# ducha-aiki/affnet

Hardware: AMD Instinct MI355X
Metric: keypoints/sec (detect+AffNet+OriNet+HardNet) per image, 2000 kp @1024x768 (higher is better)
Workload: dtype f32

## Files before the change

affnet_amd/csrc/cnn32.hip:

```cpp
#include <math.h>
#include <stdlib.h>

#include <algorithm>
#include <type_traits>

#include "common.h"

#include "cnn_mfma.h"
#include "shape_filter.h"

#define HEAD_PART_AFF 32
#define HEAD_PART_ORI 144
template <int TM>
__device__ __forceinline__ void head_partials(const float* __restrict__ hw, const f32x4 (&bias)[1], const f32x4 (&acc)[TM][1],
                                              float* __restrict__ part, int wave, int lane) {
    constexpr int MT = 4, MG = MT / TM;
    const int mg = wave % MG, ng = wave / MG;
    const int n = lane & 15, g = lane >> 4;
    const int c4 = ng * 16 + 4 * g;
    f32x4 v[TM];
#pragma unroll
    for (int i = 0; i < TM; ++i) {
        v[i] = acc[i][0] + bias[0];
        v[i].x = fmaxf(v[i].x, 0.0f); v[i].y = fmaxf(v[i].y, 0.0f); v[i].z = fmaxf(v[i].z, 0.0f); v[i].w = fmaxf(v[i].w, 0.0f);
// ... 159 lines not shown
    static constexpr int NB1 = 2, NB3 = 1;
    static constexpr int offset(int layer) { return layer == 1 ? 0 : (layer == 3 ? U1 : U1 + U3); }
    static constexpr int floats(int layer) { return layer == 1 ? U1 : (layer == 3 ? U3 : U5); }
};

__global__ __launch_bounds__(256) void wino_derive_u_kernel(const float* __restrict__ packed, int w1, int w3, int w5, float* __restrict__ U) {
    int e = blockIdx.x * 256 + threadIdx.x;
    if (e >= Wino16::PAIRS) return;
    const int l = e >= 256 + 1024 ? 5 : (e >= 256 ? 3 : 1);
    const int ch = 8 << ((l + 1) >> 1);
    const float* src = packed + (l == 5 ? w5 : (l == 3 ? w3 : w1));
    float* dst = U + Wino16::offset(l);
    e -= l == 5 ? 256 + 1024 : (l == 3 ? 256 : 0);
    const int n = (e >> 2) % ch, c = (e >> 2) / ch * 4 + (e & 3);
    float g[9], u[16];
#pragma unroll
    for (int t = 0; t < 9; ++t) g[t] = src[w_tap_index(t, c, n, ch, ch)];
    wino_weight_transform(g, u);
#pragma unroll
    for (int xi = 0; xi < 16; ++xi) dst[w_tap_index(xi, c, n, ch, ch)] = u[xi];
}

template <int CB>
struct TrunkLds {
    static constexpr int ACT = (CB / 4) * LayC0::PSG;
    static constexpr int PATCH = WP32 * WP32;
    static constexpr int RED = 256;
    static constexpr int TOTAL = ACT + PATCH + RED;
};

template <int KIND, int NW>
struct TrunkShape {
    static constexpr int CB = (KIND == AFFNET_NET_HARDNET) ? 32 : 16;
    static constexpr int NTHR = NW * 64;
    static constexpr int T1M = (CB == 16) ? 8 : 64 / NW, T1N = CB / 16;
    static constexpr int T2M = (CB == 16) ? 4 : 64 / NW, T2N = 1;
    static constexpr int T4M = (CB == 16) ? 2 : 32 / NW, T4N = 1;
    static constexpr int AREG = (NW == 8 && CB == 32) ? 128 : 48;
    static constexpr int G2 = pick_groups(CB, T2M, T2N, 32, AREG), G3 = pick_groups(2 * CB, T2M, T2N, 32, AREG);
    static constexpr int G4 = pick_groups(2 * CB, T4M, T4N, 32, AREG), G5 = pick_groups(4 * CB, T4M, T4N, 32, AREG);
};

template <int C, typename L, int NTHR>
__device__ __forceinline__ void dump_planes(const float* act, float* dst) {
    constexpr int H = L::H;
    for (int i = threadIdx.x; i < C * H * H; i += NTHR) {
        const int c = i / (H * H), r = i - c * H * H, y = r / H, x = r - y * H;
        dst[i] = act[L::at(c, y, x)];
    }
}

template <int CB>
struct SplitLays {
    typedef LayQ<16, 32, 34, CB, 0, 3> LQH;
    typedef LayQ<16, 32, 34, CB, 16, 3> LQH2;
    using LR0 = LayR<32, 32, 34, CB, 0>;
    using LR0H = LayR<16, 32, 34, CB, 0, 34>;
    using LR1 = LayR<32, 32, 34, CB, 16>;
    using LR1H = LayR<16, 32, 34, CB, 16, 34>;
    static_assert(LR0::BYTES <= TrunkLds<CB>::ACT * 4 && LR1::BYTES <= TrunkLds<CB>::ACT * 4 && LR0H::GS == LR0::GS && LR1H::GS == LR1::GS, "whole-patch split layouts");
    static_assert(LQH::BYTES <= TrunkLds<CB>::ACT * 4 && LQH2::BYTES <= TrunkLds<CB>::ACT * 4, "pre-split layouts must fit the activation buffer");
};

template <int KIND, int NW, bool STAMPS, int S3 = 0>
__global__ __launch_bounds__(NW * 64, (KIND == AFFNET_NET_HARDNET) ? NW / 4 : 4) void cnn32_trunk_kernel(CnnArgs a, PyrSrc ps) {
    static_assert(S3 == 0 || S3 == 2 || S3 == 3, "S3 = number of terms of the split arithmetic");
    using S = TrunkShape<KIND, NW>;
    constexpr int CB = S::CB, NTHR = S::NTHR;
    static_assert((CB / 4) * LayC1::PSG <= TrunkLds<CB>::ACT && (CB / 2) * LayC3::PSG <= TrunkLds<CB>::ACT, "LDS layout");
    __shared__ __attribute__((aligned(16))) float lds[TrunkLds<CB>::TOTAL];
    float* act = lds;
    float* patch = lds + TrunkLds<CB>::ACT;
    float* red = patch + TrunkLds<CB>::PATCH;
    const int n = a.count ? min(a.count[blockIdx.y], a.n_max) : a.n_max;
    const int prow = blockIdx.x + a.row_begin;
    if (KIND == AFFNET_NET_AFFNET && a.shape_cnt && blockIdx.x == 0 && threadIdx.x == 0) {
        int32_t* c = a.shape_cnt + (size_t)blockIdx.y * CNT_TOTAL;
        if (a.shape_op == 1) { c[CNT_SURVIVED] = 0; c[CNT_SURVIVED1] = 0; c[CNT_AFF_EVAL] = 0; }
        else if (a.shape_op == 2) c[CNT_SURVIVED1] = c[CNT_SURVIVED];
    }
    if (prow >= n || lazy_skip(a.skip_cnt, a.skip_n, blockIdx.y, CNT_SURVIVED)) return;
    const size_t pidx = (size_t)blockIdx.y * a.n_max + prow;
    const int tid = threadIdx.x, wave = tid >> 6, lane = tid & 63;
    if (KIND == AFFNET_NET_HARDNET) __builtin_amdgcn_s_setprio(3);
    CNN_STAMP(0);
    if (STAMPS && a.dbg_time && lane == 0) {
        a.dbg_time[((size_t)pidx * NW + wave) * 32 + 14] = __builtin_amdgcn_s_getreg((31 << 11) | 4);
        a.dbg_time[((size_t)pidx * NW + wave) * 32 + 15] = __builtin_amdgcn_s_getreg((31 << 11) | 20);
    }
    float w0[3][S::T1N];
    f32x4 bias0[S::T1N];
    conv0_load_w<NW, CB, S::T1M, S::T1N>(a.packed + a.off.w[0], a.packed + a.off.b[0], w0, bias0, wave, lane);
    f32x4 b1[1][S::T1N];
    f32x4 Ur[4];
    if constexpr (S3 == 0 && KIND == AFFNET_NET_AFFNET) prefetch_b0<NW, CB, 32, S::T1M, S::T1N, 1>(a.packed + a.off.w[1], b1, wave, lane);
    if constexpr (S3 == 0 && KIND == AFFNET_NET_ORINET) wino_prefetch_u_row<NW, CB, CB, 32, Wino16::NB1>(a.wino_u, Ur, wave, lane);

    constexpr int PPT = 1024 / NTHR;
    constexpr int RPT = 32 / PPT;
    float v[PPT];
    if (a.patches) {
        const float* src = a.patches + pidx * 1024;
#pragma unroll
        for (int q = 0; q < PPT; ++q) v[q] = src[tid + q * NTHR];
    } else {
        int o = a.ids[3 * pidx], l = a.ids[3 * pidx + 1];
        o = o < 0 ? 0 : (o >= ps.t.n_octaves ? ps.t.n_octaves - 1 : o);
        l = l < 0 ? 0 : (l >= ps.t.n_levels ? ps.t.n_levels - 1 : l);
        const float* img = ps.t.lvl[o][l] + blockIdx.y * ps.t.img_stride;
        const int h = ps.t.h[o], w = ps.t.w[o];
        const float* L = a.lafs + 6 * pidx;
        const float m = (float)(h < w ? h : w);
        const float t00 = L[0] * m, t01 = L[1] * m, t02 = L[2] * (float)w;
        const float t10 = L[3] * m, t11 = L[4] * m, t12 = L[5] * (float)h;
#pragma unroll
        for (int q = 0; q < PPT; ++q)
            v[q] = aff_sample_bilinear(img, h, w, t00, t01, t02, t10, t11, t12, ps.base[tid & 31], ps.base[(tid >> 5) + q * RPT]);
    }
    CNN_STAMP(16);
    if (tid < 4 * 33) {
        const int e = tid;
        const int y = e < 34 ? 0 : (e < 68 ? 33 : 1 + ((e - 68) >> 1)), x = e < 34 ? e : (e < 68 ? e - 34 : ((e - 68) & 1) * 33);
        patch[y * WP32 + x] = 0.0f;
    }
    if constexpr (S3 == 0) zero_halo<LayC0, NTHR>(act, CB);
    else if constexpr (S3 == 2) zero_halo_q<typename SplitLays<CB>::LR0, NTHR>(act);
    else zero_halo_q<typename SplitLays<CB>::LQH, NTHR>(act);
    float sum = 0.f;
#pragma unroll
    for (int q = 0; q < PPT; ++q) sum += v[q];
    const float mean = block_sum<NW>(sum, red) * (1.0f / 1024.0f);
    CNN_STAMP(17);
    float sq = 0.f;
#pragma unroll
    for (int q = 0; q < PPT; ++q) { v[q] -= mean; sq += v[q] * v[q]; }
    const float var = block_sum<NW>(sq, red + NW) * (1.0f / 1023.0f);
    const float sd = sqrtf(var) + 1e-7f;
    CNN_STAMP(18);
#pragma unroll
    for (int q = 0; q < PPT; ++q) patch[((tid >> 5) + q * RPT + 1) * WP32 + (tid & 31) + 1] = v[q] / sd;
    __syncthreads();
    CNN_STAMP(1);

    if constexpr (S3 == 0 && KIND == AFFNET_NET_HARDNET) {
        constexpr int T1M = S::T1M, T1N = S::T1N, T2M = S::T2M, T2N = S::T2N, T4M = S::T4M, T4N = S::T4N;
        constexpr int NB1 = (16 * 16 / 16) * (CB / 16) / NW, NB3 = (8 * 8 / 16) * (2 * CB / 16) / NW, NB5 = (4 * 4 / 16) * (4 * CB / 16) / NW;

        f32x4 Up[2][4];
        f32x4 Uw[16];
        {
            f32x4 acc[T1M][T1N];
            conv0_mfma<NW, CB, T1M, T1N>(patch, w0, bias0, acc, wave, lane);
            CNN_STAMP(19);
            store_tiles_lds<CB, LayC0, T1M, T1N, false>(act, bias0, acc, wave, lane);
            CNN_STAMP(20);
            wino_prefetch_u_pair<NW, CB, CB, 32, NB1>(a.packed + a.off.w_wino[0], Up, wave, lane);
            __syncthreads();
        }
        if (STAMPS && a.dbg_layer == 0) { dump_planes<CB, LayC0, NTHR>(act, a.dbg_out); return; }
        CNN_STAMP(2);

        f32x4 b2[S::G2][T2N];
        f32x4 bias2[T2N];
        {
            f32x4 y[NB1][4], bw[NB1];
            __builtin_amdgcn_s_setprio(0);
            conv3x3_wino_mfma_pair_rows<NW, CB, CB, LayC0, NB1>(act, a.packed + a.off.w_wino[0], Up, y, wave, lane);
            __builtin_amdgcn_s_setprio(3);
            CNN_STAMP(3);
            prefetch_b0<NW, 2 * CB, 16, T2M, T2N, S::G2>(a.packed + a.off.w[2], b2, wave, lane);
            prefetch_bias<NW, 16, T2M, T2N>(a.packed + a.off.b[2], bias2, wave, lane);
            wino_bias<NW, 32, CB, NB1>(a.packed + a.off.b[1], bw, wave, lane);
            __syncthreads();
            CNN_STAMP(21);
            zero_halo<LayC1, NTHR>(act, CB);
            wino_store_lds<CB, LayC1, NB1>(act, bw, y, wave, lane);
            CNN_STAMP(22);
            __syncthreads();
            CNN_STAMP(4);
        }
        if (STAMPS && a.dbg_layer == 1) { dump_planes<CB, LayC1, NTHR>(act, a.dbg_out); return; }

        {
            f32x4 acc[T2M][T2N];
            __builtin_amdgcn_s_setprio(0);
            conv3x3_mfma<NW, CB, 2 * CB, LayC1, 2, T2M, T2N, S::G2>(act, a.packed + a.off.w[2], b2, acc, wave, lane);
            __builtin_amdgcn_s_setprio(3);
            CNN_STAMP(5);
            wino_prefetch_u_pair<NW, 2 * CB, 2 * CB, 16, NB3>(a.packed + a.off.w_wino[1], Up, wave, lane);
            __syncthreads();
            zero_halo<LayC2, NTHR>(act, 2 * CB);
            store_tiles_lds<2 * CB, LayC2, T2M, T2N>(act, bias2, acc, wave, lane);
            __syncthreads();
            CNN_STAMP(6);
        }
        if (STAMPS && a.dbg_layer == 2) { dump_planes<2 * CB, LayC2, NTHR>(act, a.dbg_out); return; }

        f32x4 b4[S::G4][T4N];
        f32x4 bias4[T4N];
        {
            f32x4 y[NB3][4], bw[NB3];
            __builtin_amdgcn_s_setprio(0);
            conv3x3_wino_mfma_pair_rows<NW, 2 * CB, 2 * CB, LayC2, NB3>(act, a.packed + a.off.w_wino[1], Up, y, wave, lane);
            __builtin_amdgcn_s_setprio(3);
            CNN_STAMP(7);
            prefetch_b0<NW, 4 * CB, 8, T4M, T4N, S::G4>(a.packed + a.off.w[4], b4, wave, lane);
            prefetch_bias<NW, 8, T4M, T4N>(a.packed + a.off.b[4], bias4, wave, lane);
            wino_bias<NW, 16, 2 * CB, NB3>(a.packed + a.off.b[3], bw, wave, lane);
            __syncthreads();
            zero_halo<LayC3, NTHR>(act, 2 * CB);
            wino_store_lds<2 * CB, LayC3, NB3>(act, bw, y, wave, lane);
            __syncthreads();
            CNN_STAMP(8);
        }
        if (STAMPS && a.dbg_layer == 3) { dump_planes<2 * CB, LayC3, NTHR>(act, a.dbg_out); return; }

        {
            f32x4 acc[T4M][T4N];
            __builtin_amdgcn_s_setprio(0);
            conv3x3_mfma<NW, 2 * CB, 4 * CB, LayC3, 2, T4M, T4N, S::G4>(act, a.packed + a.off.w[4], b4, acc, wave, lane);
            __builtin_amdgcn_s_setprio(3);
            CNN_STAMP(9);
            wino_prefetch_u<NW, 4 * CB, 4 * CB, 8, NB5>(a.packed + a.off.w_wino[2], Uw, wave, lane);
            __syncthreads();
            zero_halo<LayC4, NTHR>(act, 4 * CB);
            store_tiles_lds<4 * CB, LayC4, T4M, T4N>(act, bias4, acc, wave, lane);
            __syncthreads();
            CNN_STAMP(10);
        }
        if (STAMPS && a.dbg_layer == 4) { dump_planes<4 * CB, LayC4, NTHR>(act, a.dbg_out); return; }

        f32x4 y[NB5][4], bw[NB5];
        __builtin_amdgcn_s_setprio(0);
        static_assert(NB5 == 1 && (4 * CB / 16) * 4096 <= TrunkLds<CB>::ACT, "conv5: one pass per wave, V of the layer fits the activation buffer");
        conv3x3_wino_mfma_shared_v<NW, 4 * CB, 4 * CB, LayC4>(act, a.packed + a.off.w_wino[2], Uw, y, wave, lane);
        __builtin_amdgcn_s_setprio(3);
        CNN_STAMP(11);
        wino_bias<NW, 8, 4 * CB, NB5>(a.packed + a.off.b[5], bw, wave, lane);
        if (!STAMPS || a.dbg_layer < 0) {
            wino_store_global<4 * CB, 8, NB5>(a.out + pidx * (64 * 4 * CB), bw, y, wave, lane);
            CNN_STAMP(13);
            return;
        }
        __syncthreads();
        wino_store_lds<4 * CB, LayC5, NB5>(act, bw, y, wave, lane);
        __syncthreads();
        CNN_STAMP(12);
        if (STAMPS && a.dbg_layer == 5) { dump_planes<4 * CB, LayC5, NTHR>(act, a.dbg_out); return; }
    } else if constexpr (S3 == 0) {
        constexpr int T1M = S::T1M, T1N = S::T1N, T2M = S::T2M, T2N = S::T2N, T4M = S::T4M, T4N = S::T4N;
        static_assert(NW == 8 && CB == 16, "Wino16 describes the 16-channel trunks on 8 waves");
        f32x4 b4[S::G4][T4N];
        f32x4 bias4[T4N];
        if constexpr (KIND == AFFNET_NET_ORINET) {
            constexpr int NB1 = Wino16::NB1, NB3 = Wino16::NB3;
            {
                f32x4 acc[T1M][T1N];
                conv0_mfma<NW, CB, T1M, T1N>(patch, w0, bias0, acc, wave, lane);
                CNN_STAMP(19);
                store_tiles_lds<CB, LayC0, T1M, T1N, false>(act, bias0, acc, wave, lane);
                CNN_STAMP(20);
                __syncthreads();
            }
            if (STAMPS && a.dbg_layer == 0) { dump_planes<CB, LayC0, NTHR>(act, a.dbg_out); return; }
            CNN_STAMP(2);

            f32x4 b2[S::G2][T2N];
            f32x4 bias2[T2N];
            {
                f32x4 y[NB1][4], bw[NB1];
                conv3x3_wino_mfma_rows<NW, CB, CB, LayC0, NB1>(act, a.wino_u, Ur, y, wave, lane);
                CNN_STAMP(3);
                prefetch_b0<NW, 2 * CB, 16, T2M, T2N, S::G2>(a.packed + a.off.w[2], b2, wave, lane);
                prefetch_bias<NW, 16, T2M, T2N>(a.packed + a.off.b[2], bias2, wave, lane);
                wino_bias<NW, 32, CB, NB1>(a.packed + a.off.b[1], bw, wave, lane);
                __syncthreads();
                CNN_STAMP(21);
                zero_halo<LayC1, NTHR>(act, CB);
                wino_store_lds<CB, LayC1, NB1>(act, bw, y, wave, lane);
                CNN_STAMP(22);
                __syncthreads();
                CNN_STAMP(4);
            }
            if (STAMPS && a.dbg_layer == 1) { dump_planes<CB, LayC1, NTHR>(act, a.dbg_out); return; }

            {
                f32x4 acc[T2M][T2N];
                conv3x3_mfma<NW, CB, 2 * CB, LayC1, 2, T2M, T2N, S::G2>(act, a.packed + a.off.w[2], b2, acc, wave, lane);
                CNN_STAMP(5);
                wino_prefetch_u_row<NW, 2 * CB, 2 * CB, 16, NB3>(a.wino_u + Wino16::offset(3), Ur, wave, lane);
                __syncthreads();
                zero_halo<LayC2, NTHR>(act, 2 * CB);
                store_tiles_lds<2 * CB, LayC2, T2M, T2N>(act, bias2, acc, wave, lane);
                __syncthreads();
                CNN_STAMP(6);
            }
            if (STAMPS && a.dbg_layer == 2) { dump_planes<2 * CB, LayC2, NTHR>(act, a.dbg_out); return; }

            {
                f32x4 y[NB3][4], bw[NB3];
                conv3x3_wino_mfma_rows<NW, 2 * CB, 2 * CB, LayC2, NB3>(act, a.wino_u + Wino16::offset(3), Ur, y, wave, lane);
                CNN_STAMP(7);
                prefetch_b0<NW, 4 * CB, 8, T4M, T4N, S::G4>(a.packed + a.off.w[4], b4, wave, lane);
                prefetch_bias<NW, 8, T4M, T4N>(a.packed + a.off.b[4], bias4, wave, lane);
                wino_bias<NW, 16, 2 * CB, NB3>(a.packed + a.off.b[3], bw, wave, lane);
                __syncthreads();
                zero_halo<LayC3, NTHR>(act, 2 * CB);
                wino_store_lds<2 * CB, LayC3, NB3>(act, bw, y, wave, lane);
                __syncthreads();
                CNN_STAMP(8);
            }
            if (STAMPS && a.dbg_layer == 3) { dump_planes<2 * CB, LayC3, NTHR>(act, a.dbg_out); return; }

        } else {
            static_assert(T1M * 8 > S::AREG, "conv1: two A sets of T1M float4 do not fit -> rolling single set (conv3x3_mfma_roll)");
            f32x4 bias1[T1N];
            {
                f32x4 acc[T1M][T1N];
                conv0_mfma<NW, CB, T1M, T1N>(patch, w0, bias0, acc, wave, lane);
                CNN_STAMP(19);
                prefetch_bias<NW, 32, T1M, T1N>(a.packed + a.off.b[1], bias1, wave, lane);
                store_tiles_lds<CB, LayC0, T1M, T1N, false>(act, bias0, acc, wave, lane);
                CNN_STAMP(20);
                __syncthreads();
            }
            if (STAMPS && a.dbg_layer == 0) { dump_planes<CB, LayC0, NTHR>(act, a.dbg_out); return; }
            CNN_STAMP(2);

            f32x4 b2[S::G2][T2N];
            f32x4 bias2[T2N];
            {
                f32x4 acc[T1M][T1N];
                conv3x3_mfma_roll<NW, CB, CB, LayC0, 1, T1M, T1N>(act, a.packed + a.off.w[1], b1, acc, wave, lane);
                CNN_STAMP(3);
                prefetch_b0<NW, 2 * CB, 16, T2M, T2N, S::G2>(a.packed + a.off.w[2], b2, wave, lane);
                prefetch_bias<NW, 16, T2M, T2N>(a.packed + a.off.b[2], bias2, wave, lane);
                __syncthreads();
                CNN_STAMP(21);
                zero_halo<LayC1, NTHR>(act, CB);
                store_tiles_lds<CB, LayC1, T1M, T1N>(act, bias1, acc, wave, lane);
                CNN_STAMP(22);
                __syncthreads();
                CNN_STAMP(4);
            }
            if (STAMPS && a.dbg_layer == 1) { dump_planes<CB, LayC1, NTHR>(act, a.dbg_out); return; }

            f32x4 b3[S::G3][T2N];
            f32x4 bias3[T2N];
            {
                f32x4 acc[T2M][T2N];
                conv3x3_mfma<NW, CB, 2 * CB, LayC1, 2, T2M, T2N, S::G2>(act, a.packed + a.off.w[2], b2, acc, wave, lane);
                CNN_STAMP(5);
                prefetch_b0<NW, 2 * CB, 16, T2M, T2N, S::G3>(a.packed + a.off.w[3], b3, wave, lane);
                prefetch_bias<NW, 16, T2M, T2N>(a.packed + a.off.b[3], bias3, wave, lane);
                __syncthreads();
                zero_halo<LayC2, NTHR>(act, 2 * CB);
                store_tiles_lds<2 * CB, LayC2, T2M, T2N>(act, bias2, acc, wave, lane);
                __syncthreads();
                CNN_STAMP(6);
            }
            if (STAMPS && a.dbg_layer == 2) { dump_planes<2 * CB, LayC2, NTHR>(act, a.dbg_out); return; }

            {
                f32x4 acc[T2M][T2N];
                conv3x3_mfma<NW, 2 * CB, 2 * CB, LayC2, 1, T2M, T2N, S::G3>(act, a.packed + a.off.w[3], b3, acc, wave, lane);
                CNN_STAMP(7);
                prefetch_b0<NW, 4 * CB, 8, T4M, T4N, S::G4>(a.packed + a.off.w[4], b4, wave, lane);
                prefetch_bias<NW, 8, T4M, T4N>(a.packed + a.off.b[4], bias4, wave, lane);
                __syncthreads();
                zero_halo<LayC3, NTHR>(act, 2 * CB);
                store_tiles_lds<2 * CB, LayC3, T2M, T2N>(act, bias3, acc, wave, lane);
                __syncthreads();
                CNN_STAMP(8);
            }
            if (STAMPS && a.dbg_layer == 3) { dump_planes<2 * CB, LayC3, NTHR>(act, a.dbg_out); return; }

        }

        f32x4 b5[S::G5][T4N];
        f32x4 bias5[T4N];
        {
            f32x4 acc[T4M][T4N];
            conv3x3_mfma<NW, 2 * CB, 4 * CB, LayC3, 2, T4M, T4N, S::G4>(act, a.packed + a.off.w[4], b4, acc, wave, lane);
            CNN_STAMP(9);
            if constexpr (KIND == AFFNET_NET_ORINET) {
                wino5_prefetch_u(a.wino_u + Wino16::offset(5), Ur, wave, lane);
            } else {
                prefetch_b0<NW, 4 * CB, 8, T4M, T4N, S::G5>(a.packed + a.off.w[5], b5, wave, lane);
                prefetch_bias<NW, 8, T4M, T4N>(a.packed + a.off.b[5], bias5, wave, lane);
            }
            __syncthreads();
// ... 900 lines not shown
```

affnet_amd/csrc/cnn_mfma.h:

```cpp
#pragma once
#include <math.h>
#include <stdlib.h>

#include "common.h"
#include "weights_layout.h"

typedef float f32x4 __attribute__((ext_vector_type(4)));

typedef __attribute__((address_space(3))) const f32x4 LdsF4;
__device__ __forceinline__ unsigned lds_byte_addr(const float* p) {
    return (unsigned)(size_t)(__attribute__((address_space(3))) const float*)p;
}
__device__ __forceinline__ f32x4 lds_read4(unsigned byte_addr) { return *(LdsF4*)(size_t)byte_addr; }

typedef unsigned u32x4 __attribute__((ext_vector_type(4)));
__device__ __forceinline__ __amdgpu_buffer_rsrc_t weight_rsrc(const float* base, int n_floats) {
    return __builtin_amdgcn_make_buffer_rsrc(const_cast<float*>(base), 0, n_floats * 4, 0x00020000);
}
__device__ __forceinline__ f32x4 buf_read4(__amdgpu_buffer_rsrc_t r, int lane_byte_off, int uniform_byte_off) {
    return __builtin_bit_cast(f32x4, __builtin_amdgcn_raw_buffer_load_b128(r, lane_byte_off, uniform_byte_off, 0));
}

template <int H_, int WP_, int PSG_>
struct Lay {
// ... 757 lines not shown
        const int p = (mg * TM + i) * 16 + m;
        const int base = (p >> 5) * WP32 + (p & 31);
        float av[3];
#pragma unroll
        for (int s3 = 0; s3 < 3; ++s3) av[s3] = patch[base + toff[s3]];
#pragma unroll
        for (int s3 = 0; s3 < 3; ++s3)
#pragma unroll
            for (int j = 0; j < TN; ++j) acc[i][j] = __builtin_amdgcn_mfma_f32_16x16x4f32(b[s3][j], av[s3], acc[i][j], 0, 0, 0);
    }
}

template <int COUT, typename LO, int TM, int TN, bool ADD_BIAS = true>
__device__ __forceinline__ void store_tiles_lds(float* act, const f32x4 (&bias)[TN], const f32x4 (&acc)[TM][TN], int wave, int lane) {
    constexpr int HOUT = LO::H;
    constexpr int MT = HOUT * HOUT / 16, MG = MT / TM;
    const int mg = wave % MG, ng = wave / MG;
    const int n = lane & 15, g = lane >> 4;
#pragma unroll
    for (int i = 0; i < TM; ++i) {
        const int p = (mg * TM + i) * 16 + n;
        const int oy = p / HOUT, ox = p - oy * HOUT;
        const int pbase = ((oy + 1) * LO::WP + ox + 1) * 4;
#pragma unroll
        for (int j = 0; j < TN; ++j) {
            const f32x4 v = ADD_BIAS ? bias_relu(acc[i][j], bias[j]) : relu4(acc[i][j]);
            *reinterpret_cast<f32x4*>(&act[((ng * TN + j) * 4 + g) * LO::PSG + pbase]) = v;
        }
    }
}

template <int COUT, int TM, int TN>
__device__ __forceinline__ void store_tiles_global(float* __restrict__ dst, const f32x4 (&bias)[TN], const f32x4 (&acc)[TM][TN],
                                                   int wave, int lane) {
    constexpr int MT = 4, MG = MT / TM;
    const int mg = wave % MG, ng = wave / MG;
    const int n = lane & 15, g = lane >> 4;
#pragma unroll
    for (int i = 0; i < TM; ++i) {
        const int p = (mg * TM + i) * 16 + n;
#pragma unroll
        for (int j = 0; j < TN; ++j) {
            const f32x4 v = bias_relu(acc[i][j], bias[j]);
            *reinterpret_cast<f32x4*>(dst + p * COUT + (ng * TN + j) * 16 + 4 * g) = v;
        }
    }
}


__device__ __forceinline__ float wadd(float a, float b) { float r = a + b; asm("" : "+v"(r)); return r; }
__device__ __forceinline__ float wsub(float a, float b) { float r = a - b; asm("" : "+v"(r)); return r; }
__device__ __forceinline__ float wmul(float a, float b) { float r = a * b; asm("" : "+v"(r)); return r; }

template <int H, int COUT, int NB>
__device__ __forceinline__ void wino_tile(int wave, int q, int m, int& ty, int& tx, int& cb) {
    constexpr int HT = H / 2, NCB = COUT / 16;
    const int p = wave * NB + q, tb = p / NCB;
    cb = p - tb * NCB;
    const int t = tb * 16 + m;
    ty = t / HT;
    tx = t - ty * HT;
}

template <int H, int COUT, int NB>
__device__ __forceinline__ int wino_u_lane(int wave, int q, int lane) {
    int ty, tx, cb;
    wino_tile<H, COUT, NB>(wave, q, lane & 15, ty, tx, cb);
    return ((lane >> 4) * COUT + cb * 16 + (lane & 15)) * 16;
}

template <int CIN, int COUT>
__device__ __forceinline__ f32x4 wino_load_u(__amdgpu_buffer_rsrc_t r, int u_lane, int k, int G, int c = 0) {
    return buf_read4(r, u_lane, (k * (CIN / 16) + G) * 16 * COUT * 4 + c * 256);
}

template <int NW, int CIN, int COUT, int H, int NB>
__device__ __forceinline__ void wino_prefetch_u(const float* __restrict__ Wu, f32x4 (&U)[16], int wave, int lane) {
    const __amdgpu_buffer_rsrc_t r = weight_rsrc(Wu, 16 * CIN * COUT);
    const int u_lane = wino_u_lane<H, COUT, NB>(wave, 0, lane);
#pragma unroll
    for (int k = 0; k < 16; ++k) U[k] = wino_load_u<CIN, COUT>(r, u_lane, k, 0);
}

__device__ __forceinline__ constexpr int wino_row_a(int i) { return i == 0 ? 0 : (i == 2 ? 2 : 1); }
__device__ __forceinline__ constexpr int wino_row_b(int i) { return i == 2 ? 1 : (i == 3 ? 3 : 2); }

template <typename LI>
__device__ __forceinline__ void wino_read_rows(unsigned ab, int i, f32x4 (&da)[4], f32x4 (&db)[4]) {
    const int ra = wino_row_a(i), rb = wino_row_b(i);
#pragma unroll
    for (int c = 0; c < 4; ++c) { da[c] = lds_read4(ab + (ra * LI::WP + c) * 16); db[c] = lds_read4(ab + (rb * LI::WP + c) * 16); }
}

__device__ __forceinline__ void wino_transform_row(int i, const f32x4 (&da)[4], const f32x4 (&db)[4], f32x4* V) {
#pragma unroll
    for (int e = 0; e < 4; ++e) {
        float t[4];
#pragma unroll
        for (int c = 0; c < 4; ++c) t[c] = i == 1 ? wadd(da[c][e], db[c][e]) : wsub(da[c][e], db[c][e]);
        V[0][e] = wsub(t[0], t[2]); V[1][e] = wadd(t[1], t[2]); V[2][e] = wsub(t[2], t[1]); V[3][e] = wsub(t[1], t[3]);
    }
}

template <typename LI>
__device__ __forceinline__ void wino_window(unsigned ab, f32x4 (&V)[16]) {
    f32x4 d[4][4];
#pragma unroll
    for (int r = 0; r < 4; ++r)
#pragma unroll
        for (int c = 0; c < 4; ++c) d[r][c] = lds_read4(ab + (r * LI::WP + c) * 16);
#pragma unroll
    for (int e = 0; e < 4; ++e) {
        float t[4][4];
#pragma unroll
        for (int c = 0; c < 4; ++c) {
            t[0][c] = wsub(d[0][c][e], d[2][c][e]); t[1][c] = wadd(d[1][c][e], d[2][c][e]);
            t[2][c] = wsub(d[2][c][e], d[1][c][e]); t[3][c] = wsub(d[1][c][e], d[3][c][e]);
        }
#pragma unroll
        for (int i = 0; i < 4; ++i) {
            V[4 * i][e] = wsub(t[i][0], t[i][2]); V[4 * i + 1][e] = wadd(t[i][1], t[i][2]);
            V[4 * i + 2][e] = wsub(t[i][2], t[i][1]); V[4 * i + 3][e] = wsub(t[i][1], t[i][3]);
        }
    }
}

__device__ __forceinline__ void wino_output(const f32x4 (&acc)[16], f32x4 (&yq)[4]) {
#pragma unroll
    for (int e = 0; e < 4; ++e) {
        float t[2][4];
#pragma unroll
        for (int j = 0; j < 4; ++j) {
            t[0][j] = wadd(wadd(acc[j][e], acc[4 + j][e]), acc[8 + j][e]);
            t[1][j] = wsub(wsub(acc[4 + j][e], acc[8 + j][e]), acc[12 + j][e]);
        }
#pragma unroll
        for (int r = 0; r < 2; ++r) {
            yq[2 * r][e] = wadd(wadd(t[r][0], t[r][1]), t[r][2]);
            yq[2 * r + 1][e] = wsub(wsub(t[r][1], t[r][2]), t[r][3]);
        }
    }
}

template <int NW, int CIN, int COUT, int H, int NB>
__device__ __forceinline__ void wino_prefetch_u_pair(const float* __restrict__ Wu, f32x4 (&U)[2][4], int wave, int lane) {
    const __amdgpu_buffer_rsrc_t r = weight_rsrc(Wu, 16 * CIN * COUT);
    const int u_lane = wino_u_lane<H, COUT, NB>(wave, 0, lane);
#pragma unroll
    for (int k = 0; k < 4; ++k)
#pragma unroll
        for (int c = 0; c < 2; ++c) U[c][k] = wino_load_u<CIN, COUT>(r, u_lane, k, 0, c);
}

template <int NW, int CIN, int COUT, typename LI, int NB>
__device__ __forceinline__ void conv3x3_wino_mfma_pair_rows(const float* act, const float* __restrict__ Wu, f32x4 (&U)[2][4], f32x4 (&y)[NB][4], int wave, int lane) {
    constexpr int H = LI::H, HT = H / 2, NGRP = CIN / 16, NSTEP = (NB / 2) * 4 * NGRP;
    static_assert(H % 2 == 0 && (HT * HT) % 16 == 0 && COUT % 16 == 0 && CIN % 16 == 0, "Winograd tiling");
    static_assert((HT * HT / 16) * (COUT / 16) == NW * NB, "the waves' passes must tile the layer exactly");
    static_assert(NB % 2 == 0 && (COUT / 16) % 2 == 0 && NSTEP % 2 == 0, "passes 2 j and 2 j + 1 must share their tile block");
    const int m = lane & 15, kq = lane >> 4;
    const __amdgpu_buffer_rsrc_t wrsrc = weight_rsrc(Wu, 16 * CIN * COUT);
    f32x4 t0[2][4], t1[2][4], acc[2][4], Va[4], Vb[4];
    auto window_addr = [&](int s) {
        const int u = s / (4 * NGRP), G = s % NGRP;
        int ty, tx, cb;
        wino_tile<H, COUT, NB>(wave, 2 * u, m, ty, tx, cb);
        unsigned ab = lds_byte_addr(act) + (((4 * G + kq) * LI::PSG + (2 * ty * LI::WP + 2 * tx) * 4) * 4);
        asm("" : "+v"(ab));
        return ab;
    };
    auto step = [&](int s, const f32x4 (&V)[4], f32x4 (&Vn)[4]) {
        const int u = s / (4 * NGRP), i = (s / NGRP) % 4, G = s % NGRP;
        const bool more = s + 1 < NSTEP;
        const int sn = more ? s + 1 : s;
        const int un = sn / (4 * NGRP), in = (sn / NGRP) % 4, Gn = sn % NGRP;
        const int u_next = wino_u_lane<H, COUT, NB>(wave, 2 * un, lane);
        unsigned abn = 0;
        if (more) abn = window_addr(sn);
        if (G == 0) {
#pragma unroll
            for (int c = 0; c < 2; ++c)
#pragma unroll
                for (int k = 0; k < 4; ++k) acc[c][k] = (f32x4){0.f, 0.f, 0.f, 0.f};
        }
        __builtin_amdgcn_sched_barrier(0);
        f32x4 da[4], db[4];
        if (more) wino_read_rows<LI>(abn, in, da, db);
#pragma unroll
        for (int k = 0; k < 4; ++k) {
#pragma unroll
            for (int s4 = 0; s4 < 4; ++s4) {
                acc[0][k] = __builtin_amdgcn_mfma_f32_16x16x4f32(U[0][k][s4], V[k][s4], acc[0][k], 0, 0, 0);
                acc[1][k] = __builtin_amdgcn_mfma_f32_16x16x4f32(U[1][k][s4], V[k][s4], acc[1][k], 0, 0, 0);
            }
            U[0][k] = wino_load_u<CIN, COUT>(wrsrc, u_next, 4 * in + k, Gn, 0);
            U[1][k] = wino_load_u<CIN, COUT>(wrsrc, u_next, 4 * in + k, Gn, 1);
        }
        if (more) {
            wino_transform_row(in, da, db, Vn);
#pragma unroll
            for (int l = 0; l < 8; ++l) {
                __builtin_amdgcn_sched_group_barrier(0x008, 1, 0);
                __builtin_amdgcn_sched_group_barrier(0x100, 1, 0);
            }
            __builtin_amdgcn_sched_group_barrier(0x020, 2, 0);
            __builtin_amdgcn_sched_group_barrier(0x008, 8, 0);
            __builtin_amdgcn_sched_group_barrier(0x020, 2, 0);
#pragma unroll
            for (int h = 0; h < 2; ++h) {
#pragma unroll
                for (int l = 0; l < 8; ++l) {
                    __builtin_amdgcn_sched_group_barrier(0x008, 1, 0);
                    __builtin_amdgcn_sched_group_barrier(0x002, 2, 0);
                }
                __builtin_amdgcn_sched_group_barrier(0x020, 2, 0);
            }
        }
        __builtin_amdgcn_sched_barrier(0);
        if (G == NGRP - 1) {
#pragma unroll
            for (int c = 0; c < 2; ++c) {
#pragma unroll
                for (int j = 0; j < 4; ++j)
#pragma unroll
                    for (int e = 0; e < 4; ++e) {
                        if (i == 0) t0[c][j][e] = acc[c][j][e];
                        else if (i == 1) { t0[c][j][e] = wadd(t0[c][j][e], acc[c][j][e]); t1[c][j][e] = acc[c][j][e]; }
                        else if (i == 2) { t0[c][j][e] = wadd(t0[c][j][e], acc[c][j][e]); t1[c][j][e] = wsub(t1[c][j][e], acc[c][j][e]); }
                        else t1[c][j][e] = wsub(t1[c][j][e], acc[c][j][e]);
                    }
                if (i == 3) {
#pragma unroll
                    for (int e = 0; e < 4; ++e) {
                        y[2 * u + c][0][e] = wadd(wadd(t0[c][0][e], t0[c][1][e]), t0[c][2][e]);
                        y[2 * u + c][1][e] = wsub(wsub(t0[c][1][e], t0[c][2][e]), t0[c][3][e]);
                        y[2 * u + c][2][e] = wadd(wadd(t1[c][0][e], t1[c][1][e]), t1[c][2][e]);
                        y[2 * u + c][3][e] = wsub(wsub(t1[c][1][e], t1[c][2][e]), t1[c][3][e]);
                    }
                }
            }
            __builtin_amdgcn_sched_barrier(0);
        }
    };
    {
        f32x4 da[4], db[4];
        wino_read_rows<LI>(window_addr(0), 0, da, db);
        wino_transform_row(0, da, db, Va);
    }
#pragma unroll
    for (int s = 0; s < NSTEP; s += 2) {
        step(s, Va, Vb);
        step(s + 1, Vb, Va);
    }
}

template <int NW, int CIN, int COUT, typename LI>
__device__ __forceinline__ void conv3x3_wino_mfma_shared_v(float* act, const float* __restrict__ Wu, f32x4 (&U)[16], f32x4 (&y)[1][4], int wave, int lane) {
    constexpr int NGRP = CIN / 16;
    static_assert(LI::H == 8 && COUT == 16 * NW && NGRP == NW, "one tile block, one channel block and one K group per wave");
    const int m = lane & 15, kq = lane >> 4;
    const __amdgpu_buffer_rsrc_t wrsrc = weight_rsrc(Wu, 16 * CIN * COUT);
    int ty, tx, cb;
    wino_tile<8, COUT, 1>(wave, 0, m, ty, tx, cb);
    const int u_lane = wino_u_lane<8, COUT, 1>(wave, 0, lane);
    f32x4 V[16];
    wino_window<LI>(lds_byte_addr(act) + ((wave * 4 + kq) * LI::PSG + (2 * ty * LI::WP + 2 * tx) * 4) * 4, V);
    __syncthreads();
    const unsigned v0 = lds_byte_addr(act) + lane * 16;
#pragma unroll
    for (int k = 0; k < 16; ++k) *reinterpret_cast<f32x4*>(&act[((wave * 16 + k) * 64 + lane) * 4]) = V[k];
    __syncthreads();
#pragma unroll
    for (int k = 0; k < 16; ++k) V[k] = lds_read4(v0 + k * 1024);
    f32x4 acc[16];
#pragma unroll
    for (int k = 0; k < 16; ++k) acc[k] = (f32x4){0.f, 0.f, 0.f, 0.f};
#pragma unroll 1
    for (int G = 0; G < NGRP; ++G) {
        const int Gn = G == NGRP - 1 ? G : G + 1;
        unsigned vb = v0 + Gn * 16 * 1024;
        asm("" : "+v"(vb));
        __builtin_amdgcn_sched_barrier(0);
#pragma unroll
        for (int k = 0; k < 16; k += 2) {
#pragma unroll
            for (int s4 = 0; s4 < 4; ++s4) {
                acc[k] = __builtin_amdgcn_mfma_f32_16x16x4f32(U[k][s4], V[k][s4], acc[k], 0, 0, 0);
                acc[k + 1] = __builtin_amdgcn_mfma_f32_16x16x4f32(U[k + 1][s4], V[k + 1][s4], acc[k + 1], 0, 0, 0);
            }
            U[k] = wino_load_u<CIN, COUT>(wrsrc, u_lane, k, Gn);
            U[k + 1] = wino_load_u<CIN, COUT>(wrsrc, u_lane, k + 1, Gn);
            V[k] = lds_read4(vb + k * 1024);
            V[k + 1] = lds_read4(vb + (k + 1) * 1024);
            __builtin_amdgcn_sched_barrier(0);
        }
    }
    wino_output(acc, y[0]);
}

template <int NW, int CIN, int COUT, int H, int NB>
__device__ __forceinline__ void wino_prefetch_u_row(const float* __restrict__ Wu, f32x4 (&U)[4], int wave, int lane) {
    const __amdgpu_buffer_rsrc_t r = weight_rsrc(Wu, 16 * CIN * COUT);
    const int u_lane = wino_u_lane<H, COUT, NB>(wave, 0, lane);
#pragma unroll
    for (int k = 0; k < 4; ++k) U[k] = wino_load_u<CIN, COUT>(r, u_lane, k, 0);
}

template <int NW, int CIN, int COUT, typename LI, int NB>
__device__ __forceinline__ void conv3x3_wino_mfma_rows(const float* act, const float* __restrict__ Wu, f32x4 (&U)[4], f32x4 (&y)[NB][4], int wave, int lane) {
    constexpr int H = LI::H, HT = H / 2, NGRP = CIN / 16, NSTEP = NB * 4 * NGRP;
    static_assert(H % 2 == 0 && (HT * HT) % 16 == 0 && COUT % 16 == 0 && CIN % 16 == 0, "Winograd tiling");
    static_assert((HT * HT / 16) * (COUT / 16) == NW * NB, "the waves' passes must tile the layer exactly");
    const int m = lane & 15, kq = lane >> 4;
    const __amdgpu_buffer_rsrc_t wrsrc = weight_rsrc(Wu, 16 * CIN * COUT);
    f32x4 t0[4], t1[4], acc[4];
#pragma unroll
    for (int s = 0; s < NSTEP; ++s) {
        const int q = s / (4 * NGRP), i = (s / NGRP) % 4, G = s % NGRP;
        const int sn = s + 1 < NSTEP ? s + 1 : s;
        const int qn = sn / (4 * NGRP), in = (sn / NGRP) % 4, Gn = sn % NGRP;
        int ty, tx, cb;
        wino_tile<H, COUT, NB>(wave, q, m, ty, tx, cb);
        const int u_next = wino_u_lane<H, COUT, NB>(wave, qn, lane);
        unsigned ab = lds_byte_addr(act) + (((4 * G + kq) * LI::PSG + (2 * ty * LI::WP + 2 * tx) * 4) * 4);
        asm("" : "+v"(ab));
        f32x4 da[4], db[4], V[4];
        wino_read_rows<LI>(ab, i, da, db);
        wino_transform_row(i, da, db, V);
        if (G == 0) {
#pragma unroll
            for (int k = 0; k < 4; ++k) acc[k] = (f32x4){0.f, 0.f, 0.f, 0.f};
        }
        __builtin_amdgcn_sched_barrier(0);
#pragma unroll
        for (int k = 0; k < 4; k += 2) {
#pragma unroll
            for (int s4 = 0; s4 < 4; ++s4) {
                acc[k] = __builtin_amdgcn_mfma_f32_16x16x4f32(U[k][s4], V[k][s4], acc[k], 0, 0, 0);
                acc[k + 1] = __builtin_amdgcn_mfma_f32_16x16x4f32(U[k + 1][s4], V[k + 1][s4], acc[k + 1], 0, 0, 0);
            }
            U[k] = wino_load_u<CIN, COUT>(wrsrc, u_next, 4 * in + k, Gn);
            U[k + 1] = wino_load_u<CIN, COUT>(wrsrc, u_next, 4 * in + k + 1, Gn);
            __builtin_amdgcn_sched_barrier(0);
        }
        if (G == NGRP - 1) {
#pragma unroll
            for (int j = 0; j < 4; ++j)
#pragma unroll
                for (int e = 0; e < 4; ++e) {
                    if (i == 0) t0[j][e] = acc[j][e];
                    else if (i == 1) { t0[j][e] = wadd(t0[j][e], acc[j][e]); t1[j][e] = acc[j][e]; }
                    else if (i == 2) { t0[j][e] = wadd(t0[j][e], acc[j][e]); t1[j][e] = wsub(t1[j][e], acc[j][e]); }
                    else t1[j][e] = wsub(t1[j][e], acc[j][e]);
                }
            if (i == 3) {
#pragma unroll
                for (int e = 0; e < 4; ++e) {
                    y[q][0][e] = wadd(wadd(t0[0][e], t0[1][e]), t0[2][e]);
                    y[q][1][e] = wsub(wsub(t0[1][e], t0[2][e]), t0[3][e]);
                    y[q][2][e] = wadd(wadd(t1[0][e], t1[1][e]), t1[2][e]);
                    y[q][3][e] = wsub(wsub(t1[1][e], t1[2][e]), t1[3][e]);
                }
            }
        }
    }
}

struct Wino5 {
    static constexpr int X = 16 * LayC4::PSG, X_FLOATS = 8 * 4 * 256;
    static constexpr int HEAD = 0;
    static constexpr int U_HALF = 8 * 4 * 16 * 64 * 4;
};
__device__ __forceinline__ void wino5_prefetch_u(const float* __restrict__ Wu, f32x4 (&U)[4], int wave, int lane) {
    const __amdgpu_buffer_rsrc_t r = weight_rsrc(Wu, 16 * 64 * 64);
    const int u_lane = ((lane >> 4) * 64 + (wave >> 1) * 16 + (lane & 15)) * 16 + (wave & 1) * Wino5::U_HALF;
#pragma unroll
    for (int k = 0; k < 4; ++k) U[k] = wino_load_u<64, 64>(r, u_lane, k, 0);
}

template <int NW, typename LI>
__device__ __forceinline__ void conv3x3_wino_mfma_half_rows(const float* act, const float* __restrict__ Wu, f32x4 (&U)[4], f32x4 (&acc)[2][4], int wave, int lane) {
    constexpr int CIN = 64, COUT = 64, NGRP = CIN / 16, NSTEP = 2 * NGRP;
    static_assert(NW == 8 && LI::H == 8, "one tile block; a wave pair per channel block");
    const int m = lane & 15, kq = lane >> 4, p = wave >> 1;
    const __amdgpu_buffer_rsrc_t wrsrc = weight_rsrc(Wu, 16 * CIN * COUT);
    const int u_lane = (kq * COUT + p * 16 + m) * 16;
    const unsigned a0 = lds_byte_addr(act) + ((kq * LI::PSG + (2 * (m >> 2) * LI::WP + 2 * (m & 3)) * 4) * 4);
    auto rows = [&](auto hc) {
        constexpr int H2 = decltype(hc)::v;
#pragma unroll
        for (int s = 0; s < NSTEP; ++s) {
            const int il = s / NGRP, i = 2 * H2 + il, G = s % NGRP;
            const int sn = s + 1 < NSTEP ? s + 1 : s;
            const int in = 2 * H2 + sn / NGRP, Gn = sn % NGRP;
            unsigned ab = a0 + 4 * G * LI::PSG * 4;
            asm("" : "+v"(ab));
            f32x4 da[4], db[4], V[4];
            wino_read_rows<LI>(ab, i, da, db);
            wino_transform_row(i, da, db, V);
            if (G == 0) {
#pragma unroll
                for (int k = 0; k < 4; ++k) acc[il][k] = (f32x4){0.f, 0.f, 0.f, 0.f};
            }
            __builtin_amdgcn_sched_barrier(0);
#pragma unroll
            for (int k = 0; k < 4; k += 2) {
#pragma unroll
                for (int s4 = 0; s4 < 4; ++s4) {
                    acc[il][k] = __builtin_amdgcn_mfma_f32_16x16x4f32(U[k][s4], V[k][s4], acc[il][k], 0, 0, 0);
                    acc[il][k + 1] = __builtin_amdgcn_mfma_f32_16x16x4f32(U[k + 1][s4], V[k + 1][s4], acc[il][k + 1], 0, 0, 0);
                }
                U[k] = wino_load_u<CIN, COUT>(wrsrc, u_lane, 4 * in + k, Gn);
                U[k + 1] = wino_load_u<CIN, COUT>(wrsrc, u_lane, 4 * in + k + 1, Gn);
                __builtin_amdgcn_sched_barrier(0);
            }
        }
    };
    if ((wave & 1) == 0) rows(IntC<0>{}); else rows(IntC<1>{});
}

__device__ __forceinline__ void wino5_combine(float* lds, const f32x4 (&acc)[2][4], f32x4 (&y)[2], int wave, int lane) {
    const int h = wave & 1;
    float* xw = lds + Wino5::X + (wave * 4 * 64 + lane) * 4;
    const float* xr = lds + Wino5::X + ((wave ^ 1) * 4 * 64 + lane) * 4;
    if (h == 0) {
#pragma unroll
        for (int j = 0; j < 4; ++j) *reinterpret_cast<f32x4*>(&xw[j * 256]) = acc[1][j];
    } else {
#pragma unroll
        for (int j = 0; j < 4; ++j) *reinterpret_cast<f32x4*>(&xw[j * 256]) = acc[0][j];
    }
    __syncthreads();
    f32x4 o[4], t[4];
#pragma unroll
    for (int j = 0; j < 4; ++j) o[j] = *reinterpret_cast<const f32x4*>(&xr[j * 256]);
    if (h == 0) {
#pragma unroll
        for (int j = 0; j < 4; ++j)
#pragma unroll
            for (int e = 0; e < 4; ++e) t[j][e] = wadd(wadd(acc[0][j][e], acc[1][j][e]), o[j][e]);
    } else {
#pragma unroll
        for (int j = 0; j < 4; ++j)
#pragma unroll
            for (int e = 0; e < 4; ++e) t[j][e] = wsub(wsub(o[j][e], acc[0][j][e]), acc[1][j][e]);
    }
#pragma unroll
    for (int e = 0; e < 4; ++e) {
        y[0][e] = wadd(wadd(t[0][e], t[1][e]), t[2][e]);
        y[1][e] = wsub(wsub(t[1][e], t[2][e]), t[3][e]);
    }
}

template <int ROW, int PIX, int GRP>
__device__ __forceinline__ void wino5_store_lds(float* dst, f32x4 bias, const f32x4 (&y)[2], int wave, int lane) {
    const int m = lane & 15, oy = 2 * (m >> 2) + (wave & 1), ox = 2 * (m & 3);
#pragma unroll
    for (int k = 0; k < 2; ++k) {
        const f32x4 v = bias_relu(y[k], bias);
        *reinterpret_cast<f32x4*>(&dst[(oy * ROW + ox + k) * PIX + ((wave >> 1) * 4 + (lane >> 4)) * GRP]) = v;
    }
}

template <int NW, int H, int COUT, int NB>
__device__ __forceinline__ void wino_bias(const float* __restrict__ bias, f32x4 (&bv)[NB], int wave, int lane) {
#pragma unroll
    for (int q = 0; q < NB; ++q) {
        int ty, tx, cb;
        wino_tile<H, COUT, NB>(wave, q, lane & 15, ty, tx, cb);
        bv[q] = *reinterpret_cast<const f32x4*>(&bias[cb * 16 + 4 * (lane >> 4)]);
    }
}

template <int COUT, typename LO, int NB>
__device__ __forceinline__ void wino_store_lds(float* act, const f32x4 (&bias)[NB], const f32x4 (&y)[NB][4], int wave, int lane) {
    const int g = lane >> 4;
#pragma unroll
    for (int q = 0; q < NB; ++q) {
        int ty, tx, cb;
        wino_tile<LO::H, COUT, NB>(wave, q, lane & 15, ty, tx, cb);
#pragma unroll
        for (int k = 0; k < 4; ++k) {
            const int oy = 2 * ty + (k >> 1), ox = 2 * tx + (k & 1);
            const f32x4 v = bias_relu(y[q][k], bias[q]);
            *reinterpret_cast<f32x4*>(&act[(cb * 4 + g) * LO::PSG + ((oy + 1) * LO::WP + ox + 1) * 4]) = v;
        }
    }
}

template <int COUT, int H, int NB>
__device__ __forceinline__ void wino_store_global(float* __restrict__ dst, const f32x4 (&bias)[NB], const f32x4 (&y)[NB][4], int wave, int lane) {
    const int g = lane >> 4;
#pragma unroll
    for (int q = 0; q < NB; ++q) {
        int ty, tx, cb;
        wino_tile<H, COUT, NB>(wave, q, lane & 15, ty, tx, cb);
#pragma unroll
        for (int k = 0; k < 4; ++k) {
            const int p = (2 * ty + (k >> 1)) * H + 2 * tx + (k & 1);
            const f32x4 v = bias_relu(y[q][k], bias[q]);
            *reinterpret_cast<f32x4*>(dst + p * COUT + cb * 16 + 4 * g) = v;
        }
    }
}
```

Before: 1.464 million.

## Issue next-layer weight and bias prefetches earlier to overlap with current conv MFMA work

```diff
diff --git a/affnet_amd/csrc/cnn32.hip b/affnet_amd/csrc/cnn32.hip
--- a/affnet_amd/csrc/cnn32.hip
+++ b/affnet_amd/csrc/cnn32.hip
@@ -335,9 +335,9 @@
             f32x4 acc[T1M][T1N];
             conv0_mfma<NW, CB, T1M, T1N>(patch, w0, bias0, acc, wave, lane);
             CNN_STAMP(19);
+            wino_prefetch_u_pair<NW, CB, CB, 32, NB1>(a.packed + a.off.w_wino[0], Up, wave, lane);
             store_tiles_lds<CB, LayC0, T1M, T1N, false>(act, bias0, acc, wave, lane);
             CNN_STAMP(20);
-            wino_prefetch_u_pair<NW, CB, CB, 32, NB1>(a.packed + a.off.w_wino[0], Up, wave, lane);
             __syncthreads();
         }
         if (STAMPS && a.dbg_layer == 0) { dump_planes<CB, LayC0, NTHR>(act, a.dbg_out); return; }
@@ -348,12 +348,10 @@
         {
             f32x4 y[NB1][4], bw[NB1];
             __builtin_amdgcn_s_setprio(0);
-            conv3x3_wino_mfma_pair_rows<NW, CB, CB, LayC0, NB1>(act, a.packed + a.off.w_wino[0], Up, y, wave, lane);
+            const WinoTailNext<NW, 32, CB, NB1, T2M, T2N, S::G2> tail{a.packed + a.off.b[1], a.packed + a.off.b[2], a.packed + a.off.w[2], bw, bias2, b2, wave, lane};
+            conv3x3_wino_mfma_pair_rows<NW, CB, CB, LayC0, NB1>(act, a.packed + a.off.w_wino[0], Up, y, wave, lane, tail);
             __builtin_amdgcn_s_setprio(3);
             CNN_STAMP(3);
-            prefetch_b0<NW, 2 * CB, 16, T2M, T2N, S::G2>(a.packed + a.off.w[2], b2, wave, lane);
-            prefetch_bias<NW, 16, T2M, T2N>(a.packed + a.off.b[2], bias2, wave, lane);
-            wino_bias<NW, 32, CB, NB1>(a.packed + a.off.b[1], bw, wave, lane);
             __syncthreads();
             CNN_STAMP(21);
             zero_halo<LayC1, NTHR>(act, CB);
@@ -366,11 +364,11 @@
 
         {
             f32x4 acc[T2M][T2N];
+            wino_prefetch_u_pair<NW, 2 * CB, 2 * CB, 16, NB3>(a.packed + a.off.w_wino[1], Up, wave, lane);
             __builtin_amdgcn_s_setprio(0);
             conv3x3_mfma<NW, CB, 2 * CB, LayC1, 2, T2M, T2N, S::G2>(act, a.packed + a.off.w[2], b2, acc, wave, lane);
             __builtin_amdgcn_s_setprio(3);
             CNN_STAMP(5);
-            wino_prefetch_u_pair<NW, 2 * CB, 2 * CB, 16, NB3>(a.packed + a.off.w_wino[1], Up, wave, lane);
             __syncthreads();
             zero_halo<LayC2, NTHR>(act, 2 * CB);
             store_tiles_lds<2 * CB, LayC2, T2M, T2N>(act, bias2, acc, wave, lane);
@@ -384,12 +382,10 @@
         {
             f32x4 y[NB3][4], bw[NB3];
             __builtin_amdgcn_s_setprio(0);
-            conv3x3_wino_mfma_pair_rows<NW, 2 * CB, 2 * CB, LayC2, NB3>(act, a.packed + a.off.w_wino[1], Up, y, wave, lane);
+            const WinoTailNext<NW, 16, 2 * CB, NB3, T4M, T4N, S::G4> tail{a.packed + a.off.b[3], a.packed + a.off.b[4], a.packed + a.off.w[4], bw, bias4, b4, wave, lane};
+            conv3x3_wino_mfma_pair_rows<NW, 2 * CB, 2 * CB, LayC2, NB3>(act, a.packed + a.off.w_wino[1], Up, y, wave, lane, tail);
             __builtin_amdgcn_s_setprio(3);
             CNN_STAMP(7);
-            prefetch_b0<NW, 4 * CB, 8, T4M, T4N, S::G4>(a.packed + a.off.w[4], b4, wave, lane);
-            prefetch_bias<NW, 8, T4M, T4N>(a.packed + a.off.b[4], bias4, wave, lane);
-            wino_bias<NW, 16, 2 * CB, NB3>(a.packed + a.off.b[3], bw, wave, lane);
             __syncthreads();
             zero_halo<LayC3, NTHR>(act, 2 * CB);
             wino_store_lds<2 * CB, LayC3, NB3>(act, bw, y, wave, lane);
@@ -400,11 +396,11 @@
 
         {
             f32x4 acc[T4M][T4N];
+            wino_prefetch_u<NW, 4 * CB, 4 * CB, 8, NB5>(a.packed + a.off.w_wino[2], Uw, wave, lane);
             __builtin_amdgcn_s_setprio(0);
             conv3x3_mfma<NW, 2 * CB, 4 * CB, LayC3, 2, T4M, T4N, S::G4>(act, a.packed + a.off.w[4], b4, acc, wave, lane);
             __builtin_amdgcn_s_setprio(3);
             CNN_STAMP(9);
-            wino_prefetch_u<NW, 4 * CB, 4 * CB, 8, NB5>(a.packed + a.off.w_wino[2], Uw, wave, lane);
             __syncthreads();
             zero_halo<LayC4, NTHR>(act, 4 * CB);
             store_tiles_lds<4 * CB, LayC4, T4M, T4N>(act, bias4, acc, wave, lane);
@@ -416,10 +412,10 @@
         f32x4 y[NB5][4], bw[NB5];
         __builtin_amdgcn_s_setprio(0);
         static_assert(NB5 == 1 && (4 * CB / 16) * 4096 <= TrunkLds<CB>::ACT, "conv5: one pass per wave, V of the layer fits the activation buffer");
+        wino_bias<NW, 8, 4 * CB, NB5>(a.packed + a.off.b[5], bw, wave, lane);
         conv3x3_wino_mfma_shared_v<NW, 4 * CB, 4 * CB, LayC4>(act, a.packed + a.off.w_wino[2], Uw, y, wave, lane);
         __builtin_amdgcn_s_setprio(3);
         CNN_STAMP(11);
-        wino_bias<NW, 8, 4 * CB, NB5>(a.packed + a.off.b[5], bw, wave, lane);
         if (!STAMPS || a.dbg_layer < 0) {
             wino_store_global<4 * CB, 8, NB5>(a.out + pidx * (64 * 4 * CB), bw, y, wave, lane);
             CNN_STAMP(13);
diff --git a/affnet_amd/csrc/cnn_mfma.h b/affnet_amd/csrc/cnn_mfma.h
--- a/affnet_amd/csrc/cnn_mfma.h
+++ b/affnet_amd/csrc/cnn_mfma.h
@@ -933,8 +933,18 @@
         for (int c = 0; c < 2; ++c) U[c][k] = wino_load_u<CIN, COUT>(r, u_lane, k, 0, c);
 }
 
-template <int NW, int CIN, int COUT, typename LI, int NB>
-__device__ __forceinline__ void conv3x3_wino_mfma_pair_rows(const float* act, const float* __restrict__ Wu, f32x4 (&U)[2][4], f32x4 (&y)[NB][4], int wave, int lane) {
+struct WinoNoTail { __device__ __forceinline__ void operator()() const {} };
+template <int NW, int H, int COUT, int NB, int TM, int TN, int GRP>
+struct WinoTailNext {
+    const float *bias, *bias_next, *w_next;
+    f32x4 (&bw)[NB];
+    f32x4 (&bv)[TN];
+    f32x4 (&b0)[GRP][TN];
+    int wave, lane;
+    __device__ __forceinline__ void operator()() const;
+};
+template <int NW, int CIN, int COUT, typename LI, int NB, typename Tail = WinoNoTail>
+__device__ __forceinline__ void conv3x3_wino_mfma_pair_rows(const float* act, const float* __restrict__ Wu, f32x4 (&U)[2][4], f32x4 (&y)[NB][4], int wave, int lane, Tail tail = Tail()) {
     constexpr int H = LI::H, HT = H / 2, NGRP = CIN / 16, NSTEP = (NB / 2) * 4 * NGRP;
     static_assert(H % 2 == 0 && (HT * HT) % 16 == 0 && COUT % 16 == 0 && CIN % 16 == 0, "Winograd tiling");
     static_assert((HT * HT / 16) * (COUT / 16) == NW * NB, "the waves' passes must tile the layer exactly");
@@ -965,6 +975,10 @@
                 for (int k = 0; k < 4; ++k) acc[c][k] = (f32x4){0.f, 0.f, 0.f, 0.f};
         }
         __builtin_amdgcn_sched_barrier(0);
+        if (!more) {
+            tail();
+            __builtin_amdgcn_sched_barrier(0);
+        }
         f32x4 da[4], db[4];
         if (more) wino_read_rows<LI>(abn, in, da, db);
 #pragma unroll
@@ -1253,6 +1267,13 @@
     }
 }
 
+template <int NW, int H, int COUT, int NB, int TM, int TN, int GRP>
+__device__ __forceinline__ void WinoTailNext<NW, H, COUT, NB, TM, TN, GRP>::operator()() const {
+    wino_bias<NW, H, COUT, NB>(bias, bw, wave, lane);
+    prefetch_bias<NW, H / 2, TM, TN>(bias_next, bv, wave, lane);
+    prefetch_b0<NW, 2 * COUT, H / 2, TM, TN, GRP>(w_next, b0, wave, lane);
+}
+
 template <int COUT, typename LO, int NB>
 __device__ __forceinline__ void wino_store_lds(float* act, const f32x4 (&bias)[NB], const f32x4 (&y)[NB][4], int wave, int lane) {
     const int g = lane >> 4;
```

Result: no change. 1.462 million (-0.1%).
